# sina-behnam/RTSDS

Hardware: AMD Instinct MI355X
Metric: images/sec/node (train step) + inference FPS@1024x512, BiSeNet 19-cls (higher is better)
Workload: dtype bf16; 1 GPU; configs[1]: BiSeNet-R18 seg-only train step (train.py:65-113); model=BiSeNet-ResNet18, global_batch=8, per_gpu_batch=8, image=3x512x1024, num_classes=19, parallelism=dp1

## Files before the change

### include/rtsds_hip.h

```cpp
#ifndef RTSDS_HIP_H
#define RTSDS_HIP_H
#include <stddef.h>
#include <stdint.h>
#ifdef __cplusplus
extern "C" {
#endif

enum { RTSDS_F32 = 0, RTSDS_BF16 = 1, RTSDS_F16 = 2  };
enum {
  RTSDS_OK = 0,
  RTSDS_ERR_SHAPE = 1,
  RTSDS_ERR_UNSUPPORTED = 2,
  RTSDS_ERR_LAUNCH = 3,
  RTSDS_ERR_WORKSPACE = 4
};
enum { RTSDS_ACT_NONE = 0, RTSDS_ACT_RELU = 1, RTSDS_ACT_LEAKY = 2, RTSDS_ACT_SIGMOID = 3 };
#define RTSDS_ACCUMULATE 0x100
#define RTSDS_INPUT_PADDED 0x400
#define RTSDS_WEIGHT_PACKED 0x800

typedef struct {
  int n, h, w, c;
  int ho, wo, k;
  int kh, kw;
// ... 93 lines not shown
int rtsds_bn_relu_maxpool_bwd(const void* dy_pool, const uint8_t* idx, const void* x, void* dx, float* dgamma,
                              float* dbeta, int n, int h, int w, int c, int ho, int wo, int p,
                              const float* gamma, const float* beta, const float* save_mean,
                              const float* save_invstd, int training, int accumulate_params, int dtype,
                              void* ws, size_t ws_bytes, void* stream);

int rtsds_nchw_to_nhwc(const float* x, void* y, int n, int c, int h, int w, int dtype, void* stream);
int rtsds_nchw_to_nhwc_pad(const float* x, void* y, int n, int c, int h, int w, int pitch, int dtype, void* stream);
int rtsds_cast(const void* src, int src_dtype, void* dst, int dst_dtype, long n, void* stream);
int rtsds_copy_channels(const void* src, int src_ld, int src_off, void* dst, int dst_ld, int dst_off,
                        long rows, int cnt, int accumulate, int dtype, void* stream);

int rtsds_act_fwd(const void* x, void* y, long n, int act, int dtype, void* stream);
int rtsds_act_bwd(const void* dy, const void* y, void* dx, long n, int act, float alpha, int dtype,
                  void* stream);

int rtsds_maxpool_fwd(const void* x, void* y, uint8_t* idx, int n, int h, int w, int c, int ho,
                      int wo, int k, int s, int p, int dtype, void* stream);
int rtsds_maxpool_bwd(const void* dy, const uint8_t* idx, void* dx, int n, int h, int w, int c,
                      int ho, int wo, int k, int s, int p, int dtype, void* stream);
size_t rtsds_gap_workspace(int n, long hw, int c);
int rtsds_gap_fwd(const void* x, void* y, int n, long hw, int c, int dtype, void* ws, size_t ws_bytes,
                  void* stream);
int rtsds_gap_bwd(const void* dy, void* dx, int n, long hw, int c, int accumulate, int dtype, void* stream);

size_t rtsds_ffm_head_eval_workspace(int n, long hw, int c);
int rtsds_ffm_head_eval(const void* f, const void* w1, const float* b1, const void* w2, const float* b2,
                        const void* w3, const float* b3, void* out, int n, long hw, int c, int dtype, void* ws,
                        size_t ws_bytes, void* stream);
int rtsds_chscale_fwd(const void* x, const void* a, void* y, int n, long hw, int c, int mode,
                      int dtype, void* stream);
int rtsds_chscale_bwd(const void* dy, const void* x, const void* a, void* dx, void* da, int n,
                      long hw, int c, int mode, int dtype, void* ws, size_t ws_bytes, void* stream);

int rtsds_bilinear_fwd(const void* x, void* y, int n, int hi, int wi, int c, int ho, int wo,
                       float scale_h, float scale_w, int y_ld, int y_off, int dtype, void* stream);
int rtsds_bilinear_fwd_scaled(const void* x, const void* s1, const void* s2, void* y, int n, int hi, int wi,
                              int c, int ho, int wo, float scale_h, float scale_w, int y_ld, int y_off,
                              int dtype, void* stream);
size_t rtsds_bilinear_bwd_workspace(int n, int hi, int wi, int c, int ho, int wo);
int rtsds_bilinear_bwd(const void* dy, void* dx, int n, int hi, int wi, int c, int ho, int wo,
                       float scale_h, float scale_w, int dy_ld, int dy_off, int dtype, void* ws,
                       size_t ws_bytes, void* stream);

int rtsds_adaptive_avgpool_fwd(const void* x, void* y, int n, int hi, int wi, int c, int ho, int wo,
                               int dtype, void* stream);
int rtsds_adaptive_avgpool_bwd(const void* dy, void* dx, int n, int hi, int wi, int c, int ho, int wo,
                               int dtype, void* stream);

int rtsds_softmax_fwd(const void* x, long sn, long sc, long shw, void* y, int y_ld, int n, long hw,
                      int c, int dtype, void* stream);
int rtsds_softmax_bwd(const void* dy, const void* y, int ld, void* dx, long sn, long sc, long shw,
                      int n, long hw, int c, int dtype, void* stream);
size_t rtsds_ce_workspace(void);
int rtsds_ce_finish(const void* ws, float* loss, void* stream);
int rtsds_ce_fwd(const void* x, long sn, long sc, long shw, const int64_t* target, float* loss, int n,
                 long hw, int c, int ignore_index, int dtype, void* ws, size_t ws_bytes, void* stream);
int rtsds_ce_bwd(const void* x, long sn, long sc, long shw, const int64_t* target,
                 const float* grad_loss, const float* count, void* dx, int n, long hw, int c,
                 int ignore_index, int dtype, void* stream);
int rtsds_bce_fwd(const float* x, const float* target, float* loss, int n, void* stream);
int rtsds_bce_bwd(const float* x, const float* target, const float* grad_loss, float* dx, int n,
                  void* stream);

int rtsds_adam_step(float* param, const void* grad, float* exp_avg, float* exp_avg_sq,
                    void* bf16_shadow, long n, float lr, float beta1, float beta2, float eps,
// ... 93 lines not shown
                       size_t ws_bytes, void* stream);
int rtsds_fda_apply(const uint8_t* src, void* dst, int dst_u8, int c, int h, int w, int b, const float* spec_src,
                    const float* amp_ref_norm, float strength, void* stream);

int rtsds_graph_split(void* graph, int max_lanes, void** handle, int* n_segments, int* n_lanes);
int rtsds_graph_lanes(void* graph, int max_lanes);
int rtsds_graph_nodes(void* graph);
int rtsds_capture_nodes(void* stream);
int rtsds_graph_split_launch(void* handle, void* stream);
int rtsds_graph_split_destroy(void* handle);

int rtsds_pooled_mlp_bwd(const void* da, const void* a, const void* h, const void* p, const void* w1,
                         const void* w2, float* dw1, float* db1, float* dw2, float* db2, void* dp,
                         int n, int c0, int c1, int c2, int accumulate, int dtype, void* stream);

int rtsds_pooled_mlp_fwd(const void* p, const void* w1, const float* b1, const void* w2, const float* b2, void* h,
                         void* a, int n, int c0, int c1, int c2, int dtype, void* stream);

int rtsds_bn_fwd_gap(const void* x, void* y, float* gap_part, int n, long hw, int c, const float* gamma, const float* beta,
                     float* running_mean, float* running_var, long long* num_batches_tracked, float* save_mean,
                     float* save_invstd, float momentum, float eps, int act, const float* stats_part, int stats_nrb,
                     int dtype, void* ws, size_t ws_bytes, void* stream);
int rtsds_ffm_att_scale(const float* part, const void* f, const void* w1, const float* b1, const void* w2, const float* b2,
                        void* pooled, void* hid, void* att, void* r, int ldr, int n, long hw, int c, int dtype,
                        void* stream);
int rtsds_ffm_att_bwd(const void* dr, const void* f, const void* a, const void* h, const void* p, const void* w1,
                      const void* w2, float* dw1, float* db1, float* dw2, float* db2, void* dp, int n, long hw, int c,
                      int accumulate, int dtype, void* ws, size_t ws_bytes, void* stream);
int rtsds_bn_bwd_ffm(const void* dr, const void* att, const void* dpooled, int n, long hw, const void* x, void* dx,
                     float* dgamma, float* dbeta, int c, const float* gamma, const float* beta, const float* save_mean,
                     const float* save_invstd, int training, int act, int accumulate_params, int dtype, void* ws,
                     size_t ws_bytes, void* stream);

#define RTSDS_ABI_VERSION 22
int rtsds_abi_version(void);

#ifdef __cplusplus
}
#endif
#endif
```

### rtsds_amd/_lib.py

```python
import ctypes
import os

import torch

_HERE = os.path.dirname(os.path.abspath(__file__))
DEFAULT_LIB_PATH = os.path.join(_HERE, "librtsds_hip.so")
ABI_VERSION = 22
LIB_PATH = os.environ.get("RTSDS_LIB") or DEFAULT_LIB_PATH

F32, BF16 = 0, 1
ACT_NONE, ACT_RELU, ACT_LEAKY, ACT_SIGMOID = 0, 1, 2, 3
ACCUMULATE = 0x100
INPUT_PADDED = 0x400
WEIGHT_PACKED = 0x800
UPCE_SET_CORRECT = 2
ERRORS = {1: "bad shape", 2: "unsupported configuration", 3: "HIP launch failure", 4: "workspace too small"}

c_int, c_long, c_float, c_size_t, c_void_p = (ctypes.c_int, ctypes.c_long, ctypes.c_float,
                                              ctypes.c_size_t, ctypes.c_void_p)


class ConvDesc(ctypes.Structure):
    _fields_ = [(n, c_int) for n in ("n", "h", "w", "c", "ho", "wo", "k", "kh", "kw", "sh", "sw",
                                     "ph", "pw", "dh", "dw", "dtype")]


class SplitReduceDesc(ctypes.Structure):
    _fields_ = [("slab", c_void_p), ("dw", c_void_p), ("slab_stride", c_long), ("nv", c_int), ("cv", c_int),
                ("cp", c_int), ("splits", c_int), ("accumulate", c_int)]


P = c_void_p
SIGNATURES = {
    "rtsds_conv2d_fwd_workspace": (c_size_t, [ctypes.POINTER(ConvDesc)]),
    "rtsds_conv2d_input_pitch": (c_int, [ctypes.POINTER(ConvDesc)]),
    "rtsds_conv2d_fwd_stats_tiles": (c_int, [ctypes.POINTER(ConvDesc)]),
    "rtsds_conv2d_fwd": (c_int, [ctypes.POINTER(ConvDesc), P, P, P, P, c_int, P, P, c_size_t, P]),
    "rtsds_conv2d_fwd_bn": (c_int, [ctypes.POINTER(ConvDesc), P, P, P, P, P, P, c_int, P, c_size_t, P]),
    "rtsds_conv2d_fwd_bn_ld": (c_int, [ctypes.POINTER(ConvDesc), P, P, P, P, P, c_long, c_int, P, c_size_t, P]),
    "rtsds_conv2d_fwd_bn_maxpool": (c_int, [ctypes.POINTER(ConvDesc), P, P, P, P, P, c_int, c_int, c_int, c_int, P,
# ... 31 lines not shown
                                 P, c_size_t, P]),
    "rtsds_bn_bwd_part": (c_int, [P, P, P, P, P, c_long, c_int, P, P, P, P, c_int, c_int, c_int, P, c_int, c_int, P,
                                  c_size_t, P]),
    "rtsds_bn_bwd": (c_int, [P, P, P, P, P, P, P, c_long, c_int, P, P, P, P, c_int, c_int, c_int, c_int,
                             P, c_size_t, P]),
    "rtsds_bn_bwd_ld": (c_int, [P, c_long, P, P, P, P, P, P, c_long, c_int, P, P, P, P, c_int, c_int, c_int, c_int,
                                P, c_size_t, P]),
    "rtsds_bn_relu_maxpool_fwd": (c_int, [P, P, P] + [c_int] * 7 + [P, P, P, P, P, P, P, c_float, c_float, c_int, P,
                                                                   c_int, c_int, P, c_size_t, P]),
    "rtsds_bn_relu_maxpool_bwd": (c_int, [P, P, P, P, P, P] + [c_int] * 7 + [P, P, P, P, c_int, c_int, c_int, P,
                                                                            c_size_t, P]),
    "rtsds_nchw_to_nhwc": (c_int, [P, P, c_int, c_int, c_int, c_int, c_int, P]),
    "rtsds_nchw_to_nhwc_pad": (c_int, [P, P, c_int, c_int, c_int, c_int, c_int, c_int, P]),
    "rtsds_cast": (c_int, [P, c_int, P, c_int, c_long, P]),
    "rtsds_ffm_head_eval_workspace": (c_size_t, [c_int, c_long, c_int]),
    "rtsds_ffm_head_eval": (c_int, [P, P, P, P, P, P, P, P, c_int, c_long, c_int, c_int, P, c_size_t, P]),
    "rtsds_graph_split": (c_int, [P, c_int, P, P, P]),
    "rtsds_graph_split_launch": (c_int, [P, P]),
    "rtsds_graph_lanes": (c_int, [P, c_int]),
    "rtsds_graph_nodes": (c_int, [P]),
    "rtsds_abi_version": (c_int, []),
    "rtsds_capture_nodes": (c_int, [P]),
    "rtsds_graph_split_destroy": (c_int, [P]),
    "rtsds_copy_channels": (c_int, [P, c_int, c_int, P, c_int, c_int, c_long, c_int, c_int, c_int, P]),
    "rtsds_act_fwd": (c_int, [P, P, c_long, c_int, c_int, P]),
    "rtsds_act_bwd": (c_int, [P, P, P, c_long, c_int, c_float, c_int, P]),
    "rtsds_maxpool_fwd": (c_int, [P, P, P] + [c_int] * 10 + [P]),
    "rtsds_maxpool_bwd": (c_int, [P, P, P] + [c_int] * 10 + [P]),
    "rtsds_gap_workspace": (c_size_t, [c_int, c_long, c_int]),
    "rtsds_gap_fwd": (c_int, [P, P, c_int, c_long, c_int, c_int, P, c_size_t, P]),
    "rtsds_gap_bwd": (c_int, [P, P, c_int, c_long, c_int, c_int, c_int, P]),
    "rtsds_chscale_fwd": (c_int, [P, P, P, c_int, c_long, c_int, c_int, c_int, P]),
    "rtsds_chscale_bwd": (c_int, [P, P, P, P, P, c_int, c_long, c_int, c_int, c_int, P, c_size_t, P]),
    "rtsds_bilinear_fwd": (c_int, [P, P] + [c_int] * 6 + [c_float, c_float, c_int, c_int, c_int, P]),
    "rtsds_bilinear_fwd_scaled": (c_int, [P, P, P, P] + [c_int] * 6 + [c_float, c_float, c_int, c_int, c_int, P]),
    "rtsds_bilinear_bwd_workspace": (c_size_t, [c_int] * 6),
    "rtsds_bilinear_bwd": (c_int, [P, P] + [c_int] * 6 + [c_float, c_float, c_int, c_int, c_int, P, c_size_t, P]),
    "rtsds_softmax_fwd": (c_int, [P, c_long, c_long, c_long, P, c_int, c_int, c_long, c_int, c_int, P]),
    "rtsds_softmax_bwd": (c_int, [P, P, c_int, P, c_long, c_long, c_long, c_int, c_long, c_int, c_int,
                                  P]),
    "rtsds_ce_workspace": (c_size_t, []),
    "rtsds_ce_fwd": (c_int, [P, c_long, c_long, c_long, P, P, c_int, c_long, c_int, c_int, c_int, P,
                             c_size_t, P]),
    "rtsds_ce_bwd": (c_int, [P, c_long, c_long, c_long, P, P, P, P, c_int, c_long, c_int, c_int, c_int,
                             P]),
    "rtsds_bce_fwd": (c_int, [P, P, P, c_int, P]),
    "rtsds_bce_bwd": (c_int, [P, P, P, P, c_int, P]),
    "rtsds_adam_step_dev": (c_int, [P, P, P, P, P, c_long, P, c_float, c_float, c_float, c_float, c_float, c_int, P]),
    "rtsds_upsoftmax_fwd": (c_int, [P, P, c_int, c_int, c_int, c_int, c_int, c_int, c_float, c_float, c_int, c_int, P]),
    "rtsds_upsoftmax_bwd_workspace": (c_size_t, [c_int, c_int, c_int, c_int, c_int, c_int]),
    "rtsds_upsoftmax_bwd": (c_int, [P, c_int, P, c_int, P, c_int, c_int, c_int, c_int, c_int, c_int, c_float, c_float,
                                    c_int, P, c_size_t, P]),
    "rtsds_upsoftmax_acc": (c_int, [P, P, P, c_int, c_int, c_int, c_int, c_int, c_int, c_float, c_float, c_int, c_int,
                                    c_int, P]),
    "rtsds_conf_hist": (c_int, [P, P, P, P, c_long, c_int, c_int, c_float, P]),
    "rtsds_pseudo_select": (c_int, [P, P, P, P, c_long, c_int, c_int, P]),
    "rtsds_upsample_pseudo": (c_int, [P, P, P, P, P] + [c_int] * 6 + [c_float, c_float, c_int, c_int, c_int, P]),
    "rtsds_upsample_paint": (c_int, [P, P, P, P, P, P] + [c_int] * 6 + [c_float, c_float, c_int, c_int, P]),
    "rtsds_slide_paint": (c_int, [P, ctypes.POINTER(c_int), c_int, P, P, P, P, P, P] + [c_int] * 8 +
                          [c_float, c_float, c_int, c_int, c_int, P]),
    "rtsds_ema_step": (c_int, [P, P, P, c_long, c_float, P]),
    "rtsds_ema_many": (c_int, [c_int, P, P, P, c_float, P]),
    "rtsds_class_presence": (c_int, [P, P, c_int, P, c_int, c_int, c_int, c_int, c_int, c_int, P]),
    "rtsds_classmix": (c_int, [P, P, P, P, P, P, P, P, c_int, P, c_int, P, P, P, P] + [c_int] * 8 + [P]),
    "rtsds_resize_aa_workspace": (c_size_t, [c_int, c_int, c_int, c_int, c_int]),
    "rtsds_resize_aa": (c_int, [P, c_int, c_int, c_int, c_int, P, c_int, c_int, c_int, c_int, P, P, c_int, c_int,
# ... 69 lines not shown
```

### rtsds_amd/csrc/chan.hip

```cpp
#include "ew_common.h"
#include "class_row.h"
#include "chan_dev.h"

template <typename T>
__global__ void __launch_bounds__(256) chan_final_kernel(const float* __restrict__ part, T* __restrict__ out, int S, int c, float scale) {
  const int img = blockIdx.y, ch = blockIdx.x * 256 + threadIdx.x;
  if (ch >= c) return;
  out[(long)img * c + ch] = from_f<T>(slice_sum(part + (long)img * S * c + ch, S, c) * scale);
}
extern "C" size_t rtsds_gap_workspace(int n, long hw, int c) {
  if (n <= 0 || hw <= 0 || c <= 0) return 256;
  return (size_t)n * chan_slices(n, hw) * c * 4 + 256;
}
template <typename T, bool DOT>
static void chan_reduce(const T* a, const T* b, T* out, int n, long hw, int c, float scale, float* part, hipStream_t st) {
  constexpr int V = VecT<T>::N;
  const int S = chan_slices(n, hw);
  if (c % V == 0)
    hipLaunchKernelGGL((chan_part_kernel<T, V, DOT>), dim3(S, n, rt_cdiv(c, 256 * V)), dim3(256), 0, st, a, b, part, hw, c);
  else
    hipLaunchKernelGGL((chan_part_kernel<T, 1, DOT>), dim3(S, n, rt_cdiv(c, 256)), dim3(256), 0, st, a, b, part, hw, c);
  hipLaunchKernelGGL(chan_final_kernel<T>, dim3(rt_cdiv(c, 256), n), dim3(256), 0, st, (const float*)part, out, S, c, scale);
}
template <typename T>
// ... 33 lines not shown
}
extern "C" int rtsds_gap_bwd(const void* dy, void* dx, int n, long hw, int c, int accumulate, int dtype, void* stream) {
  if (n <= 0 || hw <= 0 || c <= 0) return RTSDS_ERR_SHAPE;
  if (dtype == RTSDS_BF16 && c % 8 == 0) {
    const long pixels = (long)n * hw;
    hipLaunchKernelGGL(gap_bwd_vec_kernel, dim3(ew_blocks(pixels * (c / 8))), dim3(256), 0, (hipStream_t)stream, (const bf16*)dy,
                       (bf16*)dx, pixels, hw, c / 8, accumulate ? 1 : 0, 1.f / (float)hw);
    RET_LAUNCH();
  }
  DISPATCH_T(dtype, hipLaunchKernelGGL(gap_bwd_kernel<T>, dim3(ew_blocks((long)n * hw * c)), dim3(256), 0, (hipStream_t)stream, (const T*)dy, (T*)dx, n, hw, c, accumulate ? 1 : 0));
  RET_LAUNCH();
}

template <typename T>
__global__ void chscale_fwd_kernel(const T* __restrict__ x, const T* __restrict__ a, T* __restrict__ y, int n, long hw, int c, int mode) {
  const long total = (long)n * hw * c;
  GRID_STRIDE(i, total) {
    const int ch = (int)(i % c);
    const long img = i / c / hw;
    const float xv = to_f(x[i]), av = to_f(a[img * c + ch]);
    y[i] = from_f<T>(mode ? fmaf(xv, av, xv) : xv * av);
  }
}
template <typename T>
__global__ void chscale_bwd_dx_kernel(const T* __restrict__ dy, const T* __restrict__ a, T* __restrict__ dx, int n, long hw, int c, int mode) {
  const long total = (long)n * hw * c;
  GRID_STRIDE(i, total) {
    const int ch = (int)(i % c);
    const long img = i / c / hw;
    const float av = to_f(a[img * c + ch]) + (mode ? 1.f : 0.f);
    dx[i] = from_f<T>(to_f(dy[i]) * av);
  }
}
extern "C" int rtsds_chscale_fwd(const void* x, const void* a, void* y, int n, long hw, int c, int mode, int dtype, void* stream) {
  const long total = (long)n * hw * c;
  if (total <= 0) return RTSDS_ERR_SHAPE;
  DISPATCH_T(dtype, hipLaunchKernelGGL(chscale_fwd_kernel<T>, dim3(ew_blocks(total)), dim3(256), 0, (hipStream_t)stream, (const T*)x, (const T*)a, (T*)y, n, hw, c, mode));
  RET_LAUNCH();
}
static constexpr int kFfmChunk = 256;
template <typename T, int C>
__global__ void __launch_bounds__(256) ffm_head_apply_kernel(const float* __restrict__ part, const T* __restrict__ f,
                                                             const T* __restrict__ w1, const float* __restrict__ b1,
                                                             const T* __restrict__ w2, const float* __restrict__ b2,
                                                             const T* __restrict__ w3, const float* __restrict__ b3,
                                                             T* __restrict__ out, int hw) {
  typedef typename VecT<T>::v16 V16;
  constexpr int V = VecT<T>::N;
  __shared__ float wl[3][C][C + 1];
  __shared__ float gap[C], hid[C], att[C], bias3[C];
  __shared__ __attribute__((aligned(16))) T stage[kFfmChunk * C];
  const int tid = threadIdx.x, img = blockIdx.y, S = gridDim.x;
  const T* fi = f + (long)img * hw * C;
  for (int e = tid; e < C * C; e += 256) {
    const int o = e / C, i = e - o * C;
    wl[0][o][i] = to_f(w1[e]);
    wl[1][o][i] = to_f(w2[e]);
    wl[2][o][i] = to_f(w3[e]);
  }
  const int p0 = blockIdx.x * kFfmChunk, np = min(kFfmChunk, hw - p0);
  const int nvec = np * C / V;
  const V16* src = (const V16*)(fi + (long)p0 * C);
  for (int e = tid; e < nvec; e += 256) ((V16*)stage)[e] = src[e];
  if (tid < C) {
    gap[tid] = to_f(from_f<T>(slice_sum(part + (long)img * S * C + tid, S, C) * (1.f / (float)hw)));
    bias3[tid] = b3 ? b3[tid] : 0.f;
  }
  __syncthreads();
  if (tid < C) {
    float v = b1 ? b1[tid] : 0.f;
// ... 143 lines not shown
      const float x = to_f(xv[u][j]);
      o[j] = from_f<T>(fmaf(x, att[ch], x));
      ch = ch + 1 == C ? 0 : ch + 1;
    }
    dst[e] = o;
  }
  if (dense) return;
  __syncthreads();
  const int vpp = ldr / V;
  V16* out = (V16*)(r + ((long)img * hw + p0) * ldr);
  for (int e = tid; e < np * vpp; e += 256) {
    const int p = e / vpp, j0 = (e - p * vpp) * V;
    V16 o;
#pragma unroll
    for (int j = 0; j < V; ++j) o[j] = j0 + j < C ? stage[p * C + j0 + j] : from_f<T>(0.f);
    out[e] = o;
  }
}
extern "C" int rtsds_ffm_att_scale(const float* part, const void* f, const void* w1, const float* b1, const void* w2,
                                   const float* b2, void* pooled, void* hid, void* att, void* r, int ldr, int n, long hw, int c,
                                   int dtype, void* stream) {
  if (n <= 0 || n > 65535 || hw <= 0 || hw >= (1L << 31) / 64) return RTSDS_ERR_SHAPE;
  if (c != 19) return RTSDS_ERR_UNSUPPORTED;
  const int V = dtype == RTSDS_BF16 ? 8 : 4;
  if (hw % V) return RTSDS_ERR_UNSUPPORTED;
  if (ldr != c && (ldr < c || ldr % V || ldr > 64 || ((size_t)r & 15))) return RTSDS_ERR_UNSUPPORTED;
  if (!part || !f || !w1 || !w2 || !pooled || !hid || !att || !r) return RTSDS_ERR_SHAPE;
  const int S = chan_slices(n, hw);
  DISPATCH_T(dtype, hipLaunchKernelGGL((ffm_att_scale_kernel<T, 19>), dim3((int)((hw + kFfmChunk - 1) / kFfmChunk), n), dim3(256),
                                       0, (hipStream_t)stream, part, S, (const T*)f, (const T*)w1, b1, (const T*)w2, b2,
                                       (T*)pooled, (T*)hid, (T*)att, (T*)r, (int)hw, 1.f / (float)hw, ldr));
  RET_LAUNCH();
}
extern "C" int rtsds_chscale_bwd(const void* dy, const void* x, const void* a, void* dx, void* da, int n, long hw, int c, int mode,
                                 int dtype, void* ws, size_t ws_bytes, void* stream) {
  const long total = (long)n * hw * c;
  if (total <= 0) return RTSDS_ERR_SHAPE;
  if (da && ws_bytes < rtsds_gap_workspace(n, hw, c)) return RTSDS_ERR_WORKSPACE;
  hipStream_t st = (hipStream_t)stream;
  DISPATCH_T(dtype, {
    if (dx) hipLaunchKernelGGL(chscale_bwd_dx_kernel<T>, dim3(ew_blocks(total)), dim3(256), 0, st, (const T*)dy, (const T*)a, (T*)dx, n, hw, c, mode);
    if (da) chan_reduce<T, true>((const T*)dy, (const T*)x, (T*)da, n, hw, c, 1.f, (float*)ws, st);
  });
  RET_LAUNCH();
}

static const int kStageMaxC = 64;
static inline bool stage_ok(long sn, long sc, long shw, long hw, int c) {
  return sc == 1 && shw == c && sn == hw * c && c <= kStageMaxC;
}
RT_DEV long pixel_offset(long p, long hw, long sn, long shw) {
  const long img = p / hw, s = p - img * hw;
  return img * sn + s * shw;
}

template <typename RI, typename RO>
RT_DEV void px_softmax(RI x, RO y, int c) {
  const float m = row_max(x, c);
  const float iz = 1.f / row_sum_exp(x, c, m);
  for (int k = 0; k < c; ++k) y[k] = from_f<typename RO::elem>(expf(x(k) - m) * iz);
}
template <typename RG, typename RY, typename RO>
RT_DEV void px_softmax_bwd(RG g, RY y, RO dx, int c) {
  float dot = 0.f;
  for (int k = 0; k < c; ++k) dot = fmaf(g(k), y(k), dot);
  for (int k = 0; k < c; ++k) dx[k] = from_f<typename RO::elem>(y(k) * (g(k) - dot));
}
template <typename T>
__global__ void __launch_bounds__(256) softmax_fwd_staged(const T* __restrict__ x, T* __restrict__ y, long total, int c) {
  T* buf = stage_buf<T>();
  STAGE_TILES(p0, total) {
    const int np = tile_in(buf, p0, total, c, x);
    T* r = buf + threadIdx.x * c;
    if ((int)threadIdx.x < np) px_softmax(dense_row(r), dense_row(r), c);
    tile_out(y, buf, p0, np, c);
// ... 287 lines not shown
```

### rtsds_amd/csrc/chan_dev.h

```cpp
#pragma once
#include "common.h"
#include <algorithm>

static inline int chan_slices(int n, long hw) {
  return (int)std::max<long>(1, std::min<long>(hw / 32, std::max(1, 1024 / std::max(1, n))));
}

template <typename T>
struct ChanLoad {
  const T* a;
  RT_DEV float at(long o) const { return to_f(a[o]); }
  RT_DEV typename VecT<T>::v16 vec(long o) const { return *(const typename VecT<T>::v16*)(a + o); }
};

template <typename T, int VEC, bool DOT, class A>
RT_DEV void chan_part_body(const A& a, const T* __restrict__ b, float* __restrict__ part, long hw, int c, float* red) {
  const int s = blockIdx.x, S = gridDim.x, img = blockIdx.y;
  const int cbase = blockIdx.z * 256 * VEC;
  const int cl = min(c - cbase, 256 * VEC);
  const int tpr = (cl + VEC - 1) / VEC, rpi = 256 / tpr;
  const int tid = threadIdx.x, cv = tid % tpr, rg = tid / tpr;
  const int ch0 = cbase + cv * VEC;
  const long per = (hw + S - 1) / S, r0 = s * per, r1 = min(hw, r0 + per);
  float acc[VEC];
// ... 27 lines not shown
        const V16 va = a.vec(o);
        if (DOT) {
          const V16 vb = *(const V16*)(b + o);
#pragma unroll
          for (int j = 0; j < VEC; ++j) acc[j] = fmaf(to_f(va[j]), to_f(vb[j]), acc[j]);
        } else {
#pragma unroll
          for (int j = 0; j < VEC; ++j) acc[j] += to_f(va[j]);
        }
      } else {
        const float a0 = a.at(o);
        acc[0] = DOT ? fmaf(a0, to_f(b[o]), acc[0]) : acc[0] + a0;
      }
    }
  }
#pragma unroll
  for (int j = 0; j < VEC; ++j) red[tid * VEC + j] = acc[j];
  __syncthreads();
  if (rg == 0 && cv * VEC < cl) {
    for (int g = 1; g < rpi; ++g)
#pragma unroll
      for (int j = 0; j < VEC; ++j) acc[j] += red[(g * tpr + cv) * VEC + j];
#pragma unroll
    for (int j = 0; j < VEC; ++j)
      if (ch0 + j < c) part[((long)img * S + s) * c + ch0 + j] = acc[j];
  }
}
template <typename T, int VEC, bool DOT>
__global__ void __launch_bounds__(256) chan_part_kernel(const T* __restrict__ a, const T* __restrict__ b, float* __restrict__ part,
                                                        long hw, int c) {
  __shared__ float red[256 * VEC];
  chan_part_body<T, VEC, DOT>(ChanLoad<T>{a}, b, part, hw, c, red);
}
template <int U = 8>
RT_DEV float slice_sum(const float* __restrict__ p, int S, int c) {
  float s = 0.f;
  int q = 0;
  for (; q + U <= S; q += U) {
    float t[U];
#pragma unroll
    for (int u = 0; u < U; ++u) t[u] = p[(long)(q + u) * c];
#pragma unroll
    for (int u = 0; u < U; ++u) s += t[u];
  }
  for (; q < S; ++q) s += p[(long)q * c];
  return s;
}
```

### rtsds_amd/functional.py

```python
import ctypes

import numpy as np
import torch

from ._lib import ACT_RELU, ACT_SIGMOID, INPUT_PADDED, UPCE_SET_CORRECT, WEIGHT_PACKED, ConvDesc, SplitReduceDesc, lib
from .runtime import (CL, bump_params_epoch, collective, dcode, dp_world, empty_nhwc, nhwc, params_epoch,
                      register_fold, require_hip, side_enabled, side_fork, stream, workspace)

_P = lambda t: None if t is None else t.data_ptr()

CONV_PROFILE = None


def _conv_flops(d):
    return 2.0 * d.n * d.ho * d.wo * d.k * d.c * d.kh * d.kw


class _Timed:
    def __init__(self, d, tag="fwd"):
        self.d, self.tag = d, tag

    def __enter__(self):
        if CONV_PROFILE is not None:
            self.e0 = torch.cuda.Event(enable_timing=True)
# ... 1115 lines not shown

class GapFn(torch.autograd.Function):

    @staticmethod
    def forward(ctx, x, join=None):
        require_hip(x)
        x = nhwc(x)
        n, c, h, w = x.shape
        y = empty_nhwc(n, c, 1, 1, x.dtype, x.device)
        ws = workspace(lib.rtsds_gap_workspace(n, h * w, c), x.device)
        lib.rtsds_gap_fwd(_P(x), _P(y), n, h * w, c, dcode(x), _P(ws), ws.numel(), stream())
        ctx.shape = (n, c, h, w)
        ctx.join = join
        return y

    @staticmethod
    def backward(ctx, dy):
        n, c, h, w = ctx.shape
        dy = dy.contiguous()
        join = ctx.join
        acc = join is not None and join.buf is not None
        dx = join.buf if acc else empty_nhwc(n, c, h, w, dy.dtype, dy.device)
        lib.rtsds_gap_bwd(_P(dy), _P(dx), n, h * w, c, 1 if acc else 0, dcode(dy), stream())
        return (join.put(dx) if join is not None else dx), None


def global_avg_pool(x, join=None):
    return GapFn.apply(x, join)


class ChScaleFn(torch.autograd.Function):

    @staticmethod
    def forward(ctx, x, a, mode, join=None, join_a=None):
        require_hip(x, a)
        x = nhwc(x)
        a = a.contiguous()
        n, c, h, w = x.shape
        if a.dtype != x.dtype:
            a = cast(a, x.dtype)
        y = torch.empty_like(x, memory_format=CL)
        lib.rtsds_chscale_fwd(_P(x), _P(a), _P(y), n, h * w, c, mode, dcode(x), stream())
        ctx.mode = mode
        ctx.join, ctx.join_a = join, join_a
        ctx.save_for_backward(x, a)
        return y

    @staticmethod
    def backward(ctx, dy):
        x, a = ctx.saved_tensors
        n, c, h, w = x.shape
        dy = nhwc(dy)
        dx = torch.empty_like(x, memory_format=CL) if ctx.needs_input_grad[0] else None
        da = torch.empty_like(a) if ctx.needs_input_grad[1] else None
        ws = workspace(lib.rtsds_gap_workspace(n, h * w, c) if da is not None else 0, x.device)
        lib.rtsds_chscale_bwd(_P(dy), _P(x), _P(a), _P(dx), _P(da), n, h * w, c, ctx.mode,
                              dcode(x), _P(ws), ws.numel(), stream())
        if dx is not None and ctx.join is not None:
            dx = _join_add(ctx.join, dx)
        if da is not None and ctx.join_a is not None:
            da = _join_add(ctx.join_a, da)
        return dx, da, None, None, None


def channel_scale(x, a, residual=False, join=None, join_a=None):
    return ChScaleFn.apply(x, a, 1 if residual else 0, join, join_a)


def _src_scale(in_size, out_size, scale_factor):
    if scale_factor is not None and scale_factor > 0:
        return float(np.float32(1.0 / scale_factor))
    return float(np.float32(in_size) / np.float32(out_size))


class BilinearFn(torch.autograd.Function):
    @staticmethod
    def forward(ctx, x, ho, wo, sh, sw):
        require_hip(x)
        x = nhwc(x)
        n, c, hi, wi = x.shape
        y = empty_nhwc(n, c, ho, wo, x.dtype, x.device)
        lib.rtsds_bilinear_fwd(_P(x), _P(y), n, hi, wi, c, ho, wo, sh, sw, c, 0, dcode(x), stream())
        ctx.geo = (n, hi, wi, c, ho, wo, sh, sw)
        return y

    @staticmethod
    def backward(ctx, dy):
        n, hi, wi, c, ho, wo, sh, sw = ctx.geo
        dy = nhwc(dy)
        dx = empty_nhwc(n, c, hi, wi, dy.dtype, dy.device)
        ws = workspace(lib.rtsds_bilinear_bwd_workspace(n, hi, wi, c, ho, wo), dy.device)
        lib.rtsds_bilinear_bwd(_P(dy), _P(dx), n, hi, wi, c, ho, wo, sh, sw, c, 0, dcode(dy), _P(ws),
                               ws.numel(), stream())
        return dx, None, None, None, None


def interpolate_bilinear(x, size=None, scale_factor=None):
    hi, wi = x.shape[-2:]
    if size is not None:
# ... 642 lines not shown
```

### rtsds_amd/models/bisenet/build_bisenet.py

```python
import torch
from torch import nn

from rtsds_amd import functional as F
from rtsds_amd.nn import AdaptiveAvgPool2d, BatchNorm2d, Conv2d, ReLU, Sigmoid, _shadow, conv_bn, to_input
from rtsds_amd.runtime import BranchOut, branch_stream, branches_enabled

from .build_contextpath import build_contextpath


class ConvBlock(torch.nn.Module):

    def __init__(self, in_channels, out_channels, kernel_size=3, stride=2, padding=1):
        super().__init__()
        self.conv1 = Conv2d(in_channels, out_channels, kernel_size=kernel_size, stride=stride,
                            padding=padding, bias=False)
        self.bn = BatchNorm2d(out_channels)
        self.relu = ReLU()

    def forward(self, input, out=None):
        return conv_bn(self.conv1, self.bn, input, "relu", out=out)


class Spatial_path(torch.nn.Module):

    def __init__(self):
        super().__init__()
        self.convblock1 = ConvBlock(in_channels=3, out_channels=64)
        self.convblock2 = ConvBlock(in_channels=64, out_channels=128)
        self.convblock3 = ConvBlock(in_channels=128, out_channels=256)

    def forward(self, input, out=None):
        return self.convblock3(self.convblock2(self.convblock1(input)), out=out)


class AttentionRefinementModule(torch.nn.Module):

    def __init__(self, in_channels, out_channels):
        super().__init__()
        self.conv = Conv2d(in_channels, out_channels, kernel_size=1)
        self.bn = BatchNorm2d(out_channels)
        self.sigmoid = Sigmoid()
        self.in_channels = in_channels
        self.avgpool = AdaptiveAvgPool2d(output_size=(1, 1))

    def attention(self, input, pooled=None, join=None, pooled_join=None):
        if pooled is None:
            pooled = F.global_avg_pool(input, join)
        assert self.in_channels == pooled.size(1), \
            "in_channels and out_channels should all be {}".format(pooled.size(1))
        return conv_bn(self.conv, self.bn, pooled, "sigmoid", join=pooled_join)

    def forward(self, input, pooled=None, join=None, pooled_join=None):
        if pooled is None and join is None:
            join = F.GradJoin(2) if torch.is_grad_enabled() and input.requires_grad else None
        att = self.attention(input, pooled, join if pooled is None else None, pooled_join)
        return F.channel_scale(input, att, join=join)


class FeatureFusionModule(torch.nn.Module):

    fused_attention = True
    fused_head = True

    def __init__(self, num_classes, in_channels):
        super().__init__()
        self.in_channels = in_channels
        self.convblock = ConvBlock(in_channels=self.in_channels, out_channels=num_classes, stride=1)
        self.conv1 = Conv2d(num_classes, num_classes, kernel_size=1)
        self.relu = ReLU()
        self.conv2 = Conv2d(num_classes, num_classes, kernel_size=1)
        self.sigmoid = Sigmoid()
        self.avgpool = AdaptiveAvgPool2d(output_size=(1, 1))

    def forward(self, input_1, input_2=None, joins=None, reader=None):
        if input_2 is None:
            x = input_1
        else:
            parts = [input_1, *input_2] if isinstance(input_2, (tuple, list)) else [input_1, input_2]
            x = F.cat(parts, joins)
        assert self.in_channels == x.size(1), \
            "in_channels of ConvBlock should be {}".format(x.size(1))
        cb = self.convblock
        if self.fused_head and self.fused_attention and torch.is_grad_enabled() and x.is_cuda and \
                (cb.bn.training or not cb.bn.track_running_stats) and cb.bn.momentum is not None and \
                cb.conv1.in_channels != 3:
            y = cb.conv1(x, bn_stats=True)
            if F.ffm_tail_ok(y, (self.conv1, self.conv2)):
                bn = cb.bn
                track = bn.track_running_stats
# ... 80 lines not shown
                    into.record_stream(side)
                with torch.cuda.stream(side):
                    box.append(BranchOut.apply(self.saptial_path(x, out=None if into is None else (into, 0)), main, side))

            def fork():
                if self.spatial_enqueued_last:
                    ev = torch.cuda.Event()
                    ev.record(main)
                    box.append(ev)
                else:
                    side.wait_stream(main)
                    run_spatial()
            f3, f4, tail = self.context_path(x, mid=fork, tail_join=j4)
            if self.spatial_enqueued_last:
                side.wait_event(box.pop())
                run_spatial()
            sx = box[0]
            main.wait_stream(side)
            sx.record_stream(main)
        else:
            sx = self.saptial_path(x, out=None if into is None else (into, 0))
            f3, f4, tail = self.context_path(x, tail_join=j4)
        hw = sx.shape[-2:]
        heads = []
        cat = None
        infer = self.inference_fusions and not self.training and not torch.is_grad_enabled() and \
            sx.shape[1] + f3.shape[1] + f4.shape[1] == self.feature_fusion_module.in_channels
        if infer:
            att1 = self.attention_refinement_module1.attention(f3)
            att2 = self.attention_refinement_module2.attention(f4, pooled=tail)
            cat = F.concat_resized_scaled_eval(sx, ((f3, (att1,)), (f4, (att2, tail))), hw, into=into)
        if cat is None:
            cx1 = self.attention_refinement_module1(f3)
            cx2 = F.channel_scale(self.attention_refinement_module2(f4, pooled=tail, join=j4, pooled_join=jt), tail,
                                  join_a=jt)
        if infer:
            if cat is None:
                cat = F.concat_resized(sx, (cx1, cx2), hw)
            ffm = self.feature_fusion_module
            if self.with_interpolation and ffm.conv1.out_channels == 19 and \
                    (hw[0] * hw[1]) % (8 if sx.dtype == torch.bfloat16 else 4) == 0 and \
                    all(m.kernel_size == (1, 1) and m.in_channels == m.out_channels == ffm.conv1.in_channels
                        for m in (ffm.conv1, ffm.conv2, self.conv)):
                feature = ffm.convblock(cat)
                ws = [_shadow(m.weight, feature.dtype) for m in (ffm.conv1, ffm.conv2, self.conv)]
                main = F.ffm_head_eval(feature, ws[0], ffm.conv1.bias, ws[1], ffm.conv2.bias, ws[2], self.conv.bias)
                return [(main, F.upsample_geometry(main, scale_factor=8))]
            result = ffm(cat)
            if self.with_interpolation:
                main = self.conv(result)
                return [(main, F.upsample_geometry(main, scale_factor=8))]
            return [(result, None)]
        aux_on = self.training and not main_only
        j1 = j2 = None
        if aux_on:
            if torch.is_grad_enabled() and self.feature_joins:
                j1 = F.GradJoin(2, first_returns=True) if cx1.requires_grad else None
                j2 = F.GradJoin(2, first_returns=True) if cx2.requires_grad else None
            full = input.shape[-2:]
            s1 = F.interpolate_bilinear(self.supervision1(cx1, join=j1), size=hw)
            s2 = F.interpolate_bilinear(self.supervision2(cx2, join=j2), size=hw)
            aux = [(s1, F.upsample_geometry(s1, size=full)), (s2, F.upsample_geometry(s2, size=full))]
        result = self.feature_fusion_module(F.concat_resized(sx, (cx1, cx2), hw, joins=(j1, j2), into=into),
                                            reader=self.conv if self.with_interpolation else None)
        if self.with_interpolation:
            main = self.conv(result)
            heads.append((main, F.upsample_geometry(main, scale_factor=8)))
        else:
# ... 14 lines not shown
```

Baseline: 1789 images/s.

## Fuse double channel-scale in ARM2 and vectorize channel-scale kernels

Adds a chscale2 forward/backward kernel pair so the ARM2 attention scale and tail scale, previously two separate channel-scale ops, run in one pass over the feature map. The backward computes dx, da and db together with per-slice partial reductions. It also adds 16-byte vectorized forward and dx kernels and a fused dx+da backward kernel for the single channel-scale, removing separate elementwise and reduction passes. The cost is more specialized code paths with alignment and shape checks, plus slightly different bf16 rounding in the fused path.

```diff
diff --git a/include/rtsds_hip.h b/include/rtsds_hip.h
--- a/include/rtsds_hip.h
+++ b/include/rtsds_hip.h
@@ -149,6 +149,10 @@
                       int dtype, void* stream);
 int rtsds_chscale_bwd(const void* dy, const void* x, const void* a, void* dx, void* da, int n,
                       long hw, int c, int mode, int dtype, void* ws, size_t ws_bytes, void* stream);
+int rtsds_chscale2_fwd(const void* x, const void* a, const void* b, void* y, int n, long hw, int c,
+                       int dtype, void* stream);
+int rtsds_chscale2_bwd(const void* dy, const void* x, const void* a, const void* b, void* dx, void* da,
+                       void* db, int n, long hw, int c, int dtype, void* ws, size_t ws_bytes, void* stream);
 
 int rtsds_bilinear_fwd(const void* x, void* y, int n, int hi, int wi, int c, int ho, int wo,
                        float scale_h, float scale_w, int y_ld, int y_off, int dtype, void* stream);
@@ -308,7 +312,7 @@
                      const float* save_invstd, int training, int act, int accumulate_params, int dtype, void* ws,
                      size_t ws_bytes, void* stream);
 
-#define RTSDS_ABI_VERSION 22
+#define RTSDS_ABI_VERSION 23
 int rtsds_abi_version(void);
 
 #ifdef __cplusplus
diff --git a/rtsds_amd/_lib.py b/rtsds_amd/_lib.py
--- a/rtsds_amd/_lib.py
+++ b/rtsds_amd/_lib.py
@@ -5,7 +5,7 @@
 
 _HERE = os.path.dirname(os.path.abspath(__file__))
 DEFAULT_LIB_PATH = os.path.join(_HERE, "librtsds_hip.so")
-ABI_VERSION = 22
+ABI_VERSION = 23
 LIB_PATH = os.environ.get("RTSDS_LIB") or DEFAULT_LIB_PATH
 
 F32, BF16 = 0, 1
@@ -103,6 +103,8 @@
     "rtsds_gap_bwd": (c_int, [P, P, c_int, c_long, c_int, c_int, c_int, P]),
     "rtsds_chscale_fwd": (c_int, [P, P, P, c_int, c_long, c_int, c_int, c_int, P]),
     "rtsds_chscale_bwd": (c_int, [P, P, P, P, P, c_int, c_long, c_int, c_int, c_int, P, c_size_t, P]),
+    "rtsds_chscale2_fwd": (c_int, [P, P, P, P, c_int, c_long, c_int, c_int, P]),
+    "rtsds_chscale2_bwd": (c_int, [P, P, P, P, P, P, P, c_int, c_long, c_int, c_int, P, c_size_t, P]),
     "rtsds_bilinear_fwd": (c_int, [P, P] + [c_int] * 6 + [c_float, c_float, c_int, c_int, c_int, P]),
     "rtsds_bilinear_fwd_scaled": (c_int, [P, P, P, P] + [c_int] * 6 + [c_float, c_float, c_int, c_int, c_int, P]),
     "rtsds_bilinear_bwd_workspace": (c_size_t, [c_int] * 6),
diff --git a/rtsds_amd/csrc/chan.hip b/rtsds_amd/csrc/chan.hip
--- a/rtsds_amd/csrc/chan.hip
+++ b/rtsds_amd/csrc/chan.hip
@@ -89,10 +89,71 @@
     dx[i] = from_f<T>(to_f(dy[i]) * av);
   }
 }
+template <typename T, bool BWD>
+__global__ void __launch_bounds__(256) chscale_vec_kernel(const T* __restrict__ x, const T* __restrict__ a, const T* __restrict__ b,
+                                                          T* __restrict__ y, unsigned per_img, unsigned cv, int mode) {
+  typedef typename VecT<T>::v16 V16;
+  constexpr int V = VecT<T>::N;
+  const long img = blockIdx.y;
+  const V16* xi = (const V16*)x + img * per_img;
+  const V16* ai = (const V16*)a + img * cv;
+  const V16* bi = b ? (const V16*)b + img * cv : nullptr;
+  V16* yi = (V16*)y + img * per_img;
+  for (unsigned e = blockIdx.x * 256u + threadIdx.x; e < per_img; e += gridDim.x * 256u) {
+    const unsigned q = e % cv;
+    const V16 xv = xi[e], av = ai[q];
+    V16 o;
+    if (BWD) {
+      const float one = mode ? 1.f : 0.f;
+#pragma unroll
+      for (int j = 0; j < V; ++j) o[j] = from_f<T>(to_f(xv[j]) * (to_f(av[j]) + one));
+    } else {
+#pragma unroll
+      for (int j = 0; j < V; ++j) {
+        const float xf = to_f(xv[j]), af = to_f(av[j]);
+        o[j] = from_f<T>(mode ? fmaf(xf, af, xf) : xf * af);
+      }
+      if (bi) {
+        const V16 bv = bi[q];
+#pragma unroll
+        for (int j = 0; j < V; ++j) o[j] = from_f<T>(to_f(o[j]) * to_f(bv[j]));
+      }
+    }
+    yi[e] = o;
+  }
+}
+template <typename T>
+static bool chscale_vec_ok(int n, long hw, int c, std::initializer_list<const void*> ptrs) {
+  constexpr int V = VecT<T>::N;
+  if (c % V || n > 65535 || hw * (c / V) >= (1L << 31)) return false;
+  for (const void* p : ptrs)
+    if ((size_t)p & 15) return false;
+  return true;
+}
+template <typename T, bool BWD>
+static void chscale_vec(const T* x, const T* a, const T* b, T* y, int n, long hw, int c, int mode, hipStream_t st) {
+  const long per_img = hw * (c / VecT<T>::N);
+  hipLaunchKernelGGL((chscale_vec_kernel<T, BWD>), dim3(ew_blocks(per_img, 256, std::max(1, 8192 / n)), n), dim3(256), 0, st, x, a, b, y,
+                     (unsigned)per_img, (unsigned)(c / VecT<T>::N), mode);
+}
 extern "C" int rtsds_chscale_fwd(const void* x, const void* a, void* y, int n, long hw, int c, int mode, int dtype, void* stream) {
   const long total = (long)n * hw * c;
   if (total <= 0) return RTSDS_ERR_SHAPE;
-  DISPATCH_T(dtype, hipLaunchKernelGGL(chscale_fwd_kernel<T>, dim3(ew_blocks(total)), dim3(256), 0, (hipStream_t)stream, (const T*)x, (const T*)a, (T*)y, n, hw, c, mode));
+  DISPATCH_T(dtype, {
+    if (chscale_vec_ok<T>(n, hw, c, {x, a, y}))
+      chscale_vec<T, false>((const T*)x, (const T*)a, (const T*)nullptr, (T*)y, n, hw, c, mode, (hipStream_t)stream);
+    else
+      hipLaunchKernelGGL(chscale_fwd_kernel<T>, dim3(ew_blocks(total)), dim3(256), 0, (hipStream_t)stream, (const T*)x, (const T*)a, (T*)y, n, hw, c, mode);
+  });
+  RET_LAUNCH();
+}
+extern "C" int rtsds_chscale2_fwd(const void* x, const void* a, const void* b, void* y, int n, long hw, int c, int dtype,
+                                  void* stream) {
+  if (n <= 0 || hw <= 0 || c <= 0 || !x || !a || !b || !y) return RTSDS_ERR_SHAPE;
+  DISPATCH_T(dtype, {
+    if (!chscale_vec_ok<T>(n, hw, c, {x, a, b, y})) return RTSDS_ERR_UNSUPPORTED;
+    chscale_vec<T, false>((const T*)x, (const T*)a, (const T*)b, (T*)y, n, hw, c, 0, (hipStream_t)stream);
+  });
   RET_LAUNCH();
 }
 static constexpr int kFfmChunk = 256;
@@ -302,6 +363,81 @@
                                        (T*)pooled, (T*)hid, (T*)att, (T*)r, (int)hw, 1.f / (float)hw, ldr));
   RET_LAUNCH();
 }
+template <typename T, int VEC>
+struct ScaleGradLoad {
+  typedef typename VecT<T>::v16 V16;
+  const T* dy;
+  T* dx;
+  float f[VEC];
+  RT_DEV float at(long o) const { return to_f(dy[o]); }
+  RT_DEV V16 vec(long o) const {
+    const V16 g = *(const V16*)(dy + o);
+    V16 d;
+#pragma unroll
+    for (int j = 0; j < VEC; ++j) d[j] = from_f<T>(to_f(g[j]) * f[j]);
+    *(V16*)(dx + o) = d;
+    return g;
+  }
+};
+template <typename T, int VEC>
+__global__ void __launch_bounds__(256) chscale_bwd_part_kernel(const T* __restrict__ dy, const T* __restrict__ x, const T* __restrict__ a,
+                                                               T* __restrict__ dx, float* __restrict__ part, long hw, int c, int mode) {
+  typedef typename VecT<T>::v16 V16;
+  __shared__ float red[256 * VEC];
+  const V16 av = *(const V16*)(a + (long)blockIdx.y * c + chan_part_channel<VEC>(c));
+  ScaleGradLoad<T, VEC> ld{dy, dx, {}};
+  const float one = mode ? 1.f : 0.f;
+#pragma unroll
+  for (int j = 0; j < VEC; ++j) ld.f[j] = to_f(av[j]) + one;
+  chan_part_body<T, VEC, true>(ld, x, part, hw, c, red);
+}
+template <typename T, int VEC>
+struct Scale2GradRow {
+  typedef typename VecT<T>::v16 V16;
+  const T* dy;
+  const T* x;
+  T* dx;
+  float a[VEC], b[VEC];
+  RT_DEV void row(long o, float* acc_a, float* acc_b) const {
+    const V16 g = *(const V16*)(dy + o), xv = *(const V16*)(x + o);
+    V16 d;
+#pragma unroll
+    for (int j = 0; j < VEC; ++j) {
+      const float gf = to_f(g[j]), xf = to_f(xv[j]);
+      const float y1 = to_f(from_f<T>(xf * a[j]));
+      const float g1 = to_f(from_f<T>(gf * (b[j] + 0.f)));
+      d[j] = from_f<T>(g1 * (a[j] + 0.f));
+      acc_a[j] = fmaf(g1, xf, acc_a[j]);
+      acc_b[j] = fmaf(gf, y1, acc_b[j]);
+    }
+    *(V16*)(dx + o) = d;
+  }
+};
+template <typename T, int VEC>
+__global__ void __launch_bounds__(256) chscale2_bwd_part_kernel(const T* __restrict__ dy, const T* __restrict__ x, const T* __restrict__ a,
+                                                                const T* __restrict__ b, T* __restrict__ dx, float* __restrict__ part_a,
+                                                                float* __restrict__ part_b, long hw, int c) {
+  typedef typename VecT<T>::v16 V16;
+  __shared__ float red[2 * 256 * VEC];
+  const long so = (long)blockIdx.y * c + chan_part_channel<VEC>(c);
+  const V16 av = *(const V16*)(a + so), bv = *(const V16*)(b + so);
+  Scale2GradRow<T, VEC> f{dy, x, dx, {}, {}};
+#pragma unroll
+  for (int j = 0; j < VEC; ++j) {
+    f.a[j] = to_f(av[j]);
+    f.b[j] = to_f(bv[j]);
+  }
+  chan_part2_body<T, VEC>(f, part_a, part_b, hw, c, red);
+}
+template <typename T>
+__global__ void __launch_bounds__(256) chan_final2_kernel(const float* __restrict__ part0, const float* __restrict__ part1,
+                                                          T* __restrict__ out0, T* __restrict__ out1, int S, int c) {
+  const int img = blockIdx.y, ch = blockIdx.x * 256 + threadIdx.x;
+  if (ch >= c) return;
+  const float* part = blockIdx.z ? part1 : part0;
+  T* out = blockIdx.z ? out1 : out0;
+  out[(long)img * c + ch] = from_f<T>(slice_sum(part + (long)img * S * c + ch, S, c) * 1.f);
+}
 extern "C" int rtsds_chscale_bwd(const void* dy, const void* x, const void* a, void* dx, void* da, int n, long hw, int c, int mode,
                                  int dtype, void* ws, size_t ws_bytes, void* stream) {
   const long total = (long)n * hw * c;
@@ -309,8 +445,38 @@
   if (da && ws_bytes < rtsds_gap_workspace(n, hw, c)) return RTSDS_ERR_WORKSPACE;
   hipStream_t st = (hipStream_t)stream;
   DISPATCH_T(dtype, {
-    if (dx) hipLaunchKernelGGL(chscale_bwd_dx_kernel<T>, dim3(ew_blocks(total)), dim3(256), 0, st, (const T*)dy, (const T*)a, (T*)dx, n, hw, c, mode);
-    if (da) chan_reduce<T, true>((const T*)dy, (const T*)x, (T*)da, n, hw, c, 1.f, (float*)ws, st);
+    constexpr int V = VecT<T>::N;
+    if (dx && da && chscale_vec_ok<T>(n, hw, c, {dy, x, a, dx})) {
+      const int S = chan_slices(n, hw);
+      hipLaunchKernelGGL((chscale_bwd_part_kernel<T, V>), dim3(S, n, rt_cdiv(c, 256 * V)), dim3(256), 0, st, (const T*)dy,
+                         (const T*)x, (const T*)a, (T*)dx, (float*)ws, hw, c, mode);
+      hipLaunchKernelGGL(chan_final_kernel<T>, dim3(rt_cdiv(c, 256), n), dim3(256), 0, st, (const float*)ws, (T*)da, S, c, 1.f);
+    } else {
+      if (dx && chscale_vec_ok<T>(n, hw, c, {dy, a, dx}))
+        chscale_vec<T, true>((const T*)dy, (const T*)a, (const T*)nullptr, (T*)dx, n, hw, c, mode, st);
+      else if (dx)
+        hipLaunchKernelGGL(chscale_bwd_dx_kernel<T>, dim3(ew_blocks(total)), dim3(256), 0, st, (const T*)dy, (const T*)a, (T*)dx, n, hw, c, mode);
+      if (da) chan_reduce<T, true>((const T*)dy, (const T*)x, (T*)da, n, hw, c, 1.f, (float*)ws, st);
+    }
+  });
+  RET_LAUNCH();
+}
+extern "C" int rtsds_chscale2_bwd(const void* dy, const void* x, const void* a, const void* b, void* dx, void* da, void* db, int n,
+                                  long hw, int c, int dtype, void* ws, size_t ws_bytes, void* stream) {
+  if (n <= 0 || hw <= 0 || c <= 0 || !dy || !x || !a || !b || !dx || !da || !db) return RTSDS_ERR_SHAPE;
+  const size_t set = (size_t)n * chan_slices(n, hw) * c;
+  if (ws_bytes < 2 * set * 4 || ((size_t)ws & 15)) return RTSDS_ERR_WORKSPACE;
+  hipStream_t st = (hipStream_t)stream;
+  DISPATCH_T(dtype, {
+    constexpr int V = VecT<T>::N;
+    if (!chscale_vec_ok<T>(n, hw, c, {dy, x, a, b, dx})) return RTSDS_ERR_UNSUPPORTED;
+    const int S = chan_slices(n, hw);
+    float* pa = (float*)ws;
+    float* pb = pa + set;
+    hipLaunchKernelGGL((chscale2_bwd_part_kernel<T, V>), dim3(S, n, rt_cdiv(c, 256 * V)), dim3(256), 0, st, (const T*)dy, (const T*)x,
+                       (const T*)a, (const T*)b, (T*)dx, pa, pb, hw, c);
+    hipLaunchKernelGGL(chan_final2_kernel<T>, dim3(rt_cdiv(c, 256), n, 2), dim3(256), 0, st, (const float*)pa, (const float*)pb, (T*)da,
+                       (T*)db, S, c);
   });
   RET_LAUNCH();
 }
diff --git a/rtsds_amd/csrc/chan_dev.h b/rtsds_amd/csrc/chan_dev.h
--- a/rtsds_amd/csrc/chan_dev.h
+++ b/rtsds_amd/csrc/chan_dev.h
@@ -83,6 +83,51 @@
   __shared__ float red[256 * VEC];
   chan_part_body<T, VEC, DOT>(ChanLoad<T>{a}, b, part, hw, c, red);
 }
+template <int VEC>
+RT_DEV int chan_part_channel(int c) {
+  const int cbase = blockIdx.z * 256 * VEC;
+  const int tpr = (min(c - cbase, 256 * VEC) + VEC - 1) / VEC;
+  return cbase + (threadIdx.x % tpr) * VEC;
+}
+template <typename T, int VEC, class F>
+RT_DEV void chan_part2_body(const F& f, float* __restrict__ part0, float* __restrict__ part1, long hw, int c, float* red) {
+  const int s = blockIdx.x, S = gridDim.x, img = blockIdx.y;
+  const int cbase = blockIdx.z * 256 * VEC;
+  const int cl = min(c - cbase, 256 * VEC);
+  const int tpr = (cl + VEC - 1) / VEC, rpi = 256 / tpr;
+  const int tid = threadIdx.x, cv = tid % tpr, rg = tid / tpr;
+  const int ch0 = cbase + cv * VEC;
+  const long per = (hw + S - 1) / S, r0 = s * per, r1 = min(hw, r0 + per);
+  float acc0[VEC], acc1[VEC];
+#pragma unroll
+  for (int j = 0; j < VEC; ++j) acc0[j] = acc1[j] = 0.f;
+  if (rg < rpi) {
+    const long base = (long)img * hw * c + ch0;
+#pragma unroll 2
+    for (long r = r0 + rg; r < r1; r += rpi) f.row(base + r * c, acc0, acc1);
+  }
+  float* red1 = red + 256 * VEC;
+#pragma unroll
+  for (int j = 0; j < VEC; ++j) {
+    red[tid * VEC + j] = acc0[j];
+    red1[tid * VEC + j] = acc1[j];
+  }
+  __syncthreads();
+  if (rg == 0 && cv * VEC < cl) {
+    for (int g = 1; g < rpi; ++g)
+#pragma unroll
+      for (int j = 0; j < VEC; ++j) {
+        acc0[j] += red[(g * tpr + cv) * VEC + j];
+        acc1[j] += red1[(g * tpr + cv) * VEC + j];
+      }
+    const long o = ((long)img * S + s) * c + ch0;
+#pragma unroll
+    for (int j = 0; j < VEC; ++j) {
+      part0[o + j] = acc0[j];
+      part1[o + j] = acc1[j];
+    }
+  }
+}
 template <int U = 8>
 RT_DEV float slice_sum(const float* __restrict__ p, int S, int c) {
   float s = 0.f;
diff --git a/rtsds_amd/functional.py b/rtsds_amd/functional.py
--- a/rtsds_amd/functional.py
+++ b/rtsds_amd/functional.py
@@ -1171,7 +1171,7 @@
 class ChScaleFn(torch.autograd.Function):
 
     @staticmethod
-    def forward(ctx, x, a, mode, join=None, join_a=None):
+    def forward(ctx, x, a, mode, join=None, join_a=None, fused=True):
         require_hip(x, a)
         x = nhwc(x)
         a = a.contiguous()
@@ -1181,7 +1181,7 @@
         y = torch.empty_like(x, memory_format=CL)
         lib.rtsds_chscale_fwd(_P(x), _P(a), _P(y), n, h * w, c, mode, dcode(x), stream())
         ctx.mode = mode
-        ctx.join, ctx.join_a = join, join_a
+        ctx.join, ctx.join_a, ctx.fused = join, join_a, fused
         ctx.save_for_backward(x, a)
         return y
 
@@ -1193,17 +1193,62 @@
         dx = torch.empty_like(x, memory_format=CL) if ctx.needs_input_grad[0] else None
         da = torch.empty_like(a) if ctx.needs_input_grad[1] else None
         ws = workspace(lib.rtsds_gap_workspace(n, h * w, c) if da is not None else 0, x.device)
-        lib.rtsds_chscale_bwd(_P(dy), _P(x), _P(a), _P(dx), _P(da), n, h * w, c, ctx.mode,
-                              dcode(x), _P(ws), ws.numel(), stream())
+        for gx, ga in ((dx, da),) if ctx.fused else ((dx, None), (None, da)):
+            if gx is not None or ga is not None:
+                lib.rtsds_chscale_bwd(_P(dy), _P(x), _P(a), _P(gx), _P(ga), n, h * w, c, ctx.mode,
+                                      dcode(x), _P(ws), ws.numel(), stream())
         if dx is not None and ctx.join is not None:
             dx = _join_add(ctx.join, dx)
         if da is not None and ctx.join_a is not None:
             da = _join_add(ctx.join_a, da)
-        return dx, da, None, None, None
-
-
-def channel_scale(x, a, residual=False, join=None, join_a=None):
-    return ChScaleFn.apply(x, a, 1 if residual else 0, join, join_a)
+        return dx, da, None, None, None, None
+
+
+def channel_scale(x, a, residual=False, join=None, join_a=None, fused=True):
+    return ChScaleFn.apply(x, a, 1 if residual else 0, join, join_a, fused)
+
+
+class ChScale2Fn(torch.autograd.Function):
+
+    @staticmethod
+    def forward(ctx, x, a, b, join=None, join_b=None):
+        require_hip(x, a, b)
+        x = nhwc(x)
+        n, c, h, w = x.shape
+        a, b = (cast(t.contiguous(), x.dtype) for t in (a, b))
+        y = torch.empty_like(x, memory_format=CL)
+        lib.rtsds_chscale2_fwd(_P(x), _P(a), _P(b), _P(y), n, h * w, c, dcode(x), stream())
+        ctx.join, ctx.join_b = join, join_b
+        ctx.save_for_backward(x, a, b)
+        return y
+
+    @staticmethod
+    def backward(ctx, dy):
+        x, a, b = ctx.saved_tensors
+        n, c, h, w = x.shape
+        dy = nhwc(dy)
+        if dy.dtype != x.dtype:
+            dy = cast(dy, x.dtype)
+        dx = torch.empty_like(x, memory_format=CL)
+        da, db = torch.empty_like(a), torch.empty_like(b)
+        ws = workspace(2 * lib.rtsds_gap_workspace(n, h * w, c), x.device)
+        lib.rtsds_chscale2_bwd(_P(dy), _P(x), _P(a), _P(b), _P(dx), _P(da), _P(db), n, h * w, c, dcode(x),
+                               _P(ws), ws.numel(), stream())
+        db = _join_add(ctx.join_b, db) if ctx.needs_input_grad[2] else None
+        dx = _join_add(ctx.join, dx) if ctx.needs_input_grad[0] else None
+        return dx, (da if ctx.needs_input_grad[1] else None), db, None, None
+
+
+def channel_scale2_ok(x, a, b):
+    if x.dim() != 4 or not x.is_cuda or x.dtype not in (torch.bfloat16, torch.float32):
+        return False
+    n, c = x.shape[0], x.shape[1]
+    return c % (8 if x.dtype == torch.bfloat16 else 4) == 0 and n <= 65535 and \
+        all(t.dtype == x.dtype and tuple(t.shape) == (n, c, 1, 1) for t in (a, b))
+
+
+def channel_scale2(x, a, b, join=None, join_b=None):
+    return ChScale2Fn.apply(x, a, b, join, join_b)
 
 
 def _src_scale(in_size, out_size, scale_factor):
diff --git a/rtsds_amd/models/bisenet/build_bisenet.py b/rtsds_amd/models/bisenet/build_bisenet.py
--- a/rtsds_amd/models/bisenet/build_bisenet.py
+++ b/rtsds_amd/models/bisenet/build_bisenet.py
@@ -34,6 +34,8 @@
 
 
 class AttentionRefinementModule(torch.nn.Module):
+
+    fused_train = True
 
     def __init__(self, in_channels, out_channels):
         super().__init__()
@@ -54,7 +56,16 @@
         if pooled is None and join is None:
             join = F.GradJoin(2) if torch.is_grad_enabled() and input.requires_grad else None
         att = self.attention(input, pooled, join if pooled is None else None, pooled_join)
-        return F.channel_scale(input, att, join=join)
+        return F.channel_scale(input, att, join=join, fused=self.fused_train)
+
+    def forward_scaled(self, input, scale, pooled, join=None, pooled_join=None, scale_join=None):
+        if self.fused_train and torch.is_grad_enabled():
+            att = self.attention(input, pooled, None, pooled_join)
+            if F.channel_scale2_ok(input, att, scale):
+                return F.channel_scale2(input, att, scale, join=join, join_b=scale_join)
+            return F.channel_scale(F.channel_scale(input, att, join=join), scale, join_a=scale_join)
+        return F.channel_scale(self(input, pooled=pooled, join=join, pooled_join=pooled_join), scale,
+                               join_a=scale_join, fused=self.fused_train)
 
 
 class FeatureFusionModule(torch.nn.Module):
@@ -201,8 +212,8 @@
             cat = F.concat_resized_scaled_eval(sx, ((f3, (att1,)), (f4, (att2, tail))), hw, into=into)
         if cat is None:
             cx1 = self.attention_refinement_module1(f3)
-            cx2 = F.channel_scale(self.attention_refinement_module2(f4, pooled=tail, join=j4, pooled_join=jt), tail,
-                                  join_a=jt)
+            cx2 = self.attention_refinement_module2.forward_scaled(f4, tail, pooled=tail, join=j4, pooled_join=jt,
+                                                                   scale_join=jt)
         if infer:
             if cat is None:
                 cat = F.concat_resized(sx, (cx1, cx2), hw)
```

Result: faster. 1814 images/s, median of 6 (+1.4%).
